# marcin-ochman/modular-slam

Hardware: AMD Instinct MI355X
Metric: ORB keypoints extracted+matched /sec, 640×480 RGB-D, 1/2/4/8 GPU; HBM GB/s vs roofline (higher is better)
Workload: dtype u8

## Files before the change

### include/mslam_hip.h

```cpp
#ifndef MSLAM_HIP_H_
#define MSLAM_HIP_H_

#include <stddef.h>
#include <stdint.h>

#ifdef __cplusplus
extern "C" {
#endif

#define MSLAM_HIP_ABI_VERSION 5

enum
{
    MSLAM_HIP_OK = 0,
    MSLAM_HIP_E_INVALID = 1,
    MSLAM_HIP_E_RUNTIME = 2,
    MSLAM_HIP_E_CAPACITY = 3,
    MSLAM_HIP_E_NO_VOCABULARY = 4,
    MSLAM_HIP_E_FORMAT = 5,
    MSLAM_HIP_E_NO_MODEL = 6
};

typedef struct mslam_hip_ctx mslam_hip_ctx;

// ... 327 lines not shown
                         int* best );

typedef struct
{
    int32_t n_matches, n_correspondences, n_inliers, status;
    double rvec[3], tvec[3], R[9];
    int32_t tracked;
    int32_t keyframe_required;
    int32_t keyframe_added;
    int32_t n_entry, n_inherited;
    int32_t vote_best, vote_best_count;
} mslam_hip_track_result;
int mslam_hip_track(mslam_hip_ctx* ctx, const uint8_t* desc, const float* xy, int n, const uint16_t* depth, int width,
                    int height, float factor, double fx, double fy, double cx, double cy, int ref_id,
                    const int32_t* vote_ids, int n_vote, double ratio, int iterations, double reprojection_error,
                    uint64_t seed, int use_extrinsic_guess, const double* rvec, const double* tvec,
                    int min_matched_points , int new_keyframe_min_landmarks , int new_id ,
                    double z_max , mslam_hip_track_result* out, int32_t* vote_counts ,
                    int32_t* pair_from, int32_t* pair_to, uint8_t* inliers, int pair_stride,
                    int32_t* entry_src, int32_t* entry_kp, int entry_capacity);

typedef mslam_hip_track_result mslam_hip_track_window_result;
int mslam_hip_track_window(mslam_hip_ctx* ctx, const uint8_t* desc, const float* xy, const int32_t* n, int stride,
                           const uint16_t* depth, int S, int width, int height, float factor, double fx, double fy, double cx,
                           double cy, int ref_id, const int32_t* vote_ids, int n_vote, int ref_vote_pos, double ratio,
                           int iterations, double reprojection_error, uint64_t seed, int use_extrinsic_guess,
                           const double* rvec, const double* tvec, int min_matched_points, int new_keyframe_min_landmarks,
                           int new_id, double z_max, mslam_hip_track_window_result* out , int* first_event,
                           int32_t* vote_counts , int32_t* entry_src, int32_t* entry_kp,
                           int entry_capacity);
int mslam_hip_track_window_dev(mslam_hip_ctx* ctx, int first_frame, int n_frames, double fx, double fy, double cx, double cy,
                               int ref_id, const int32_t* vote_ids, int n_vote, int ref_vote_pos, double ratio, int iterations,
                               double reprojection_error, uint64_t seed, int use_extrinsic_guess, const double* rvec,
                               const double* tvec, int min_matched_points, int new_keyframe_min_landmarks, int new_id,
                               double z_max, mslam_hip_track_window_result* out , int* first_event,
                               int32_t* vote_counts, int32_t* entry_src, int32_t* entry_kp, int entry_capacity);

enum
{
    MSLAM_HIP_DBG_PYRAMID = 0,
    MSLAM_HIP_DBG_BLURRED = 1,
    MSLAM_HIP_DBG_CANDIDATES = 2,
    MSLAM_HIP_DBG_SELECTED = 3,
    MSLAM_HIP_DBG_CELLS = 4,
    MSLAM_HIP_DBG_FORMS = 5,
    MSLAM_HIP_DBG_QUAD_DIRECT = 6
};
int mslam_hip_level_geometry(mslam_hip_ctx* ctx, int* widths, int* heights, float* scales);
int mslam_hip_debug_read(mslam_hip_ctx* ctx, int what, int frame, int level, void* dst, size_t dst_bytes,
                         size_t* n_items);

int mslam_hip_debug_counts(mslam_hip_ctx* ctx, int what, int32_t* out, int n_frames);

int mslam_hip_copy_to_host(mslam_hip_ctx* ctx, void* dst_host, const void* src_dev, size_t bytes);

int mslam_hip_set_profiling(mslam_hip_ctx* ctx, int enable);
int mslam_hip_get_stage_times(mslam_hip_ctx* ctx, const char** names, float* ms, int cap, int* n);

#ifdef __cplusplus
}
#endif
#endif
```

### modular-slam_amd/__init__.py

```python
import ctypes as C
import os
import subprocess

import numpy as np

_HERE = os.path.dirname(os.path.abspath(__file__))
LIB_PATH = os.path.join(_HERE, "libmslam_hip.so")

OK, E_INVALID, E_RUNTIME, E_CAPACITY, E_NO_VOCABULARY, E_FORMAT, E_NO_MODEL = range(7)
DBG_PYRAMID, DBG_BLURRED, DBG_CANDIDATES, DBG_SELECTED, DBG_CELLS, DBG_FORMS, DBG_QUAD_DIRECT = range(7)
QUAD_DIRECT_MAX_CANDIDATES = 1024
MATCHER_AUTO, MATCHER_POPCOUNT = 0, 1
DETECTOR_DISTRIBUTED, DETECTOR_CV_ORB = 0, 1
BOW_ASSIGN_TREE, BOW_ASSIGN_FLAT = 0, 1
CV_ORDER_LIBSTDCXX, CV_ORDER_RASTER = 0, 1
POSE_GRAPH_MAX_KEYFRAMES, POSE_GRAPH_MAX_EDGES = 1024, 65536
POSE_GRAPH_MAX_KEYFRAMES_SPARSE, POSE_GRAPH_MAX_ENVELOPE_BLOCKS = 16384, 1048576
PG_SOLVER_DENSE, PG_SOLVER_SPARSE = 0, 1
_PG_SOLVER_NAMES = {"dense": PG_SOLVER_DENSE, "sparse": PG_SOLVER_SPARSE}
PG_ORDER_NATURAL, PG_ORDER_RCM = 0, 1
BA_GLOBAL_MAX_KEYFRAMES, BA_GLOBAL_MAX_KEYFRAMES_SPARSE = 1024, 16384
BA_GLOBAL_SOLVER_DENSE, BA_GLOBAL_SOLVER_SPARSE = 0, 1
CULL_MAX_ENTRIES = 4096
BA_LOSS_NONE, BA_LOSS_HUBER, BA_LOSS_CAUCHY = 0, 1, 2
_BA_LOSS_NAMES = {"none": BA_LOSS_NONE, "huber": BA_LOSS_HUBER, "cauchy": BA_LOSS_CAUCHY}
UNION_DESC_RECENT, UNION_DESC_DISTINCTIVE = 0, 1
_UNION_DESC_NAMES = {"recent": UNION_DESC_RECENT, "distinctive": UNION_DESC_DISTINCTIVE}

ABI_SYMBOLS = [
    "mslam_hip_default_params", "mslam_hip_abi_version", "mslam_hip_create", "mslam_hip_destroy",
    "mslam_hip_last_error", "mslam_hip_sync", "mslam_hip_detect", "mslam_hip_detect_batch_dev",
    "mslam_hip_get_batch_view", "mslam_hip_match", "mslam_hip_match_knn2", "mslam_hip_match_batch_dev",
    "mslam_hip_bow_load", "mslam_hip_bow_info", "mslam_hip_bow_words", "mslam_hip_bow_transform",
    "mslam_hip_bow_score", "mslam_hip_bow_db_add", "mslam_hip_bow_db_query", "mslam_hip_bow_db_clear",
    "mslam_hip_bow_batch_dev", "mslam_hip_get_bow_view", "mslam_hip_bow_cross_score_dev", "mslam_hip_level_geometry", "mslam_hip_debug_read",
    "mslam_hip_set_profiling", "mslam_hip_get_stage_times", "mslam_hip_copy_to_host", "mslam_hip_backproject", "mslam_hip_backproject_batch_dev",
    "mslam_hip_get_points_view", "mslam_hip_set_matcher", "mslam_hip_get_matcher",
    "mslam_hip_bow_pack_dev", "mslam_hip_bow_cross_score_packed_dev", "mslam_hip_debug_counts",
    "mslam_hip_last_match_kernel",
    "mslam_hip_join_matcher", "mslam_hip_bow_db_remove", "mslam_hip_bow_set_assignment",
    "mslam_hip_bow_db_reserve", "mslam_hip_bow_db_size", "mslam_hip_qlz_decompress",
    "mslam_hip_pnp_ransac", "mslam_hip_pnp_batch_dev", "mslam_hip_get_pnp_view", "mslam_hip_pnp_set_confidence", "mslam_hip_pack_batch_dev", "mslam_hip_packed_capacity",
    "mslam_hip_set_cv_keypoint_order", "mslam_hip_pnp_min_mse", "mslam_hip_pnp_min_mse_batch_dev",
    "mslam_hip_kf_add", "mslam_hip_kf_add_from_batch_dev", "mslam_hip_kf_remove", "mslam_hip_kf_clear", "mslam_hip_kf_size",
    "mslam_hip_kf_reserve", "mslam_hip_kf_read", "mslam_hip_relocalize",
    "mslam_hip_kf_visible", "mslam_hip_track", "mslam_hip_track_window", "mslam_hip_track_window_dev",
    "mslam_hip_kf_add_ids", "mslam_hip_kf_read_ids", "mslam_hip_kf_covisible", "mslam_hip_kf_union", "mslam_hip_kf_union_dev",
    "mslam_hip_match_guided_knn2", "mslam_hip_match_guided", "mslam_hip_set_guided_match", "mslam_hip_get_guided_match",
    "mslam_hip_bundle_adjust", "mslam_hip_bundle_adjust_global", "mslam_hip_kf_update_world", "mslam_hip_pose_graph",
    "mslam_hip_kf_fuse_search", "mslam_hip_kf_replace_ids", "mslam_hip_kf_fuse",
    "mslam_hip_kf_fuse_search_multi", "mslam_hip_kf_fuse_multi",
    "mslam_hip_kf_remove_observations",
    "mslam_hip_kf_observers", "mslam_hip_kf_cull_search", "mslam_hip_kf_cull",
    "mslam_hip_kf_remove_landmarks", "mslam_hip_kf_cull_landmarks_search", "mslam_hip_kf_cull_landmarks",
    "mslam_hip_set_ba_loss", "mslam_hip_get_ba_loss",
    "mslam_hip_set_union_descriptor", "mslam_hip_get_union_descriptor",
    "mslam_hip_set_pose_graph_solver", "mslam_hip_get_pose_graph_solver", "mslam_hip_pose_graph_analyze",
    "mslam_hip_set_ba_global_solver", "mslam_hip_get_ba_global_solver", "mslam_hip_bundle_adjust_global_analyze",
]


class MslamHipError(RuntimeError):
    def __init__(self, code, msg):
        super().__init__("mslam_hip error %d: %s" % (code, msg))
        self.code = code


class Params(C.Structure):
    _fields_ = [("width", C.c_int32), ("height", C.c_int32), ("max_batch", C.c_int32), ("n_levels", C.c_int32),
                ("scale_factor", C.c_float), ("ini_fast_thr", C.c_int32), ("min_fast_thr", C.c_int32),
                ("min_node_area", C.c_uint32), ("max_keypoints", C.c_int32), ("max_candidates", C.c_int32),
                ("device", C.c_int32), ("stream", C.c_void_p), ("detector", C.c_int32), ("n_features", C.c_int32),
                ("edge_threshold", C.c_int32)]


class BatchView(C.Structure):
    _fields_ = [("n_frames", C.c_int32), ("capacity", C.c_int32), ("xy", C.c_void_p), ("desc", C.c_void_p),
                ("octave", C.c_void_p), ("angle", C.c_void_p), ("response", C.c_void_p), ("count", C.c_void_p),
                ("match_from", C.c_void_p), ("match_to", C.c_void_p), ("match_count", C.c_void_p)]


class PointsView(C.Structure):
    _fields_ = [("capacity", C.c_int32), ("xyz", C.c_void_p), ("valid", C.c_void_p)]


class PackedHeader(C.Structure):
    _fields_ = [("n_frames", C.c_int32), ("total_keypoints", C.c_int32), ("total_matches", C.c_int32), ("with_points", C.c_int32),
                ("off_kp_offset", C.c_uint64), ("off_match_offset", C.c_uint64), ("off_xy", C.c_uint64), ("off_desc", C.c_uint64),
                ("off_octave", C.c_uint64), ("off_angle", C.c_uint64), ("off_response", C.c_uint64), ("off_xyz", C.c_uint64),
                ("off_valid", C.c_uint64), ("off_match_from", C.c_uint64), ("off_match_to", C.c_uint64), ("bytes", C.c_uint64),
                ("fits", C.c_int32), ("pad", C.c_int32)]


def unpack_batch(buf):
    h = PackedHeader.from_buffer_copy(bytes(buf[:C.sizeof(PackedHeader)]))
    if not h.fits:
        raise MslamHipError(E_CAPACITY, "packed results need %d bytes" % h.bytes)
    nk, nm, nf = h.total_keypoints, h.total_matches, h.n_frames

    def arr(off, dt, n, *shape):
        return np.frombuffer(buf, dt, n, int(off)).reshape((-1,) + shape) if shape else np.frombuffer(buf, dt, n, int(off))
    out = {"n_frames": nf, "bytes": int(h.bytes),
           "kp_offset": arr(h.off_kp_offset, np.int32, nf + 1), "match_offset": arr(h.off_match_offset, np.int32, nf + 1),
           "xy": arr(h.off_xy, np.float32, 2 * nk, 2), "desc": arr(h.off_desc, np.uint8, 32 * nk, 32),
           "octave": arr(h.off_octave, np.int32, nk), "angle": arr(h.off_angle, np.float32, nk),
           "response": arr(h.off_response, np.float32, nk),
           "match_from": arr(h.off_match_from, np.int32, nm), "match_to": arr(h.off_match_to, np.int32, nm)}
    if h.with_points:
        out["xyz"] = arr(h.off_xyz, np.float64, 3 * nk, 3)
        out["valid"] = arr(h.off_valid, np.uint8, nk)
    return out
# ... 887 lines not shown
    def bow_pack_dev(self, k_max, d_out):
        self._chk(self.L.mslam_hip_bow_pack_dev(self._h, int(k_max), C.c_void_p(d_out)))

    def bow_cross_score_packed_dev(self, d_sets, n_sets, self_set, n_frames, k_max, d_scores, stream=None):
        self._chk(self.L.mslam_hip_bow_cross_score_packed_dev(self._h, C.c_void_p(d_sets), int(n_sets), int(self_set),
                                                              int(n_frames), int(k_max), C.c_void_p(d_scores),
                                                              C.c_void_p(stream)))

    def bow_view(self):
        v = BowView()
        self._chk(self.L.mslam_hip_get_bow_view(self._h, C.byref(v)))
        return v

    def level_geometry(self):
        n = self.params.n_levels
        w = (C.c_int * 16)()
        h = (C.c_int * 16)()
        s = (C.c_float * 16)()
        self._chk(self.L.mslam_hip_level_geometry(self._h, w, h, s))
        return list(w[:n]), list(h[:n]), np.array(s[:n], np.float32)

    def debug_image(self, what, frame, level):
        w, h, _ = self.level_geometry()
        out = np.empty((h[level], w[level]), np.uint8)
        n = C.c_size_t(0)
        self._chk(self.L.mslam_hip_debug_read(self._h, what, frame, level, _p(out), C.c_size_t(out.size), C.byref(n)))
        return out

    def debug_keypoints(self, what, frame, level):
        out = np.empty((self.params.max_candidates, 3), np.float32)
        n = C.c_size_t(0)
        self._chk(self.L.mslam_hip_debug_read(self._h, what, frame, level, _p(out), C.c_size_t(out.nbytes),
                                              C.byref(n)))
        return out[:n.value].copy()

    def debug_cells(self, level):
        out = np.empty((2048, 6), np.int32)
        n = C.c_size_t(0)
        self._chk(self.L.mslam_hip_debug_read(self._h, DBG_CELLS, 0, level, _p(out), C.c_size_t(out.nbytes),
                                              C.byref(n)))
        return out[:n.value].copy()

    def debug_forms(self):
        out = np.zeros(2, np.int32)
        n = C.c_size_t(0)
        self._chk(self.L.mslam_hip_debug_read(self._h, DBG_FORMS, 0, 0, _p(out), C.c_size_t(out.nbytes), C.byref(n)))
        return int(out[0]), int(out[1])

    def debug_quad_direct_levels(self):
        out = np.zeros(1, np.uint32)
        n = C.c_size_t(0)
        self._chk(self.L.mslam_hip_debug_read(self._h, DBG_QUAD_DIRECT, 0, 0, _p(out), C.c_size_t(out.nbytes), C.byref(n)))
        return [bool((int(out[0]) >> l) & 1) for l in range(self.params.n_levels)]

    def debug_counts(self, what, n_frames):
        out = np.zeros((max(n_frames, 1), self.params.n_levels), np.int32)
        self._chk(self.L.mslam_hip_debug_counts(self._h, int(what), _p(out), int(out.shape[0])))
        return out[:n_frames]

    def set_profiling(self, enable):
        self._chk(self.L.mslam_hip_set_profiling(self._h, int(enable)))

    def stage_times(self, cap=256):
        names = (C.c_char_p * cap)()
        ms = (C.c_float * cap)()
        n = C.c_int(0)
        self._chk(self.L.mslam_hip_get_stage_times(self._h, names, ms, cap, C.byref(n)))
        return [(names[i].decode(), ms[i]) for i in range(n.value)]


def qlz_decompress(data, n_packets, capacity=None):
    src = np.frombuffer(bytes(data), np.uint8)
    cap = capacity if capacity is not None else 10000 * n_packets + 16
    dst = np.empty(max(cap, 1), np.uint8)
    n = C.c_size_t(0)
    L = lib()
    L.mslam_hip_qlz_decompress.argtypes = [C.c_void_p, C.c_size_t, C.c_uint32, C.c_void_p, C.c_size_t, C.POINTER(C.c_size_t)]
    rc = L.mslam_hip_qlz_decompress(_p(src), src.size, int(n_packets), _p(dst), dst.size, C.byref(n))
    if rc != OK:
        raise MslamHipError(rc, "qlz_decompress failed")
    return dst[:n.value].tobytes()


class RgbFrame:

    def __init__(self, data, width, height):
        self.data = np.ascontiguousarray(data, np.uint8).reshape(height, width, 3)
        self.size = (width, height)


class OrbKeypoint:
    __slots__ = ("id", "coordinates", "descriptor")

    def __init__(self, id, coordinates, descriptor):
        self.id, self.coordinates, self.descriptor = id, coordinates, descriptor


class HipOrbDetector:

    def __init__(self, width=640, height=480, **kw):
        self.ctx = Context(width=width, height=height, **kw)

    def detect(self, sensorData):
        r = self.ctx.detect(sensorData.data)
        return [OrbKeypoint(i, (float(x), float(y)), d) for i, ((x, y), d) in enumerate(zip(r["xy"].astype(np.float64),
                                                                                          r["desc"]))]
# ... 801 lines not shown
```

### modular-slam_amd/csrc/api.hip

```cpp
#include "context.hpp"

#include <cfloat>
#include <climits>
#include <cmath>
#include <cstdio>
#include <cstring>
#include <cstdlib>
#include <algorithm>

using namespace mslam;

static thread_local std::string g_create_error;

#define ENTER(c)                                                                                                       \
    do                                                                                                                 \
    {                                                                                                                  \
        if(!(c))                                                                                                       \
            return MSLAM_HIP_E_INVALID;                                                                                \
        MSLAM_CHK(c, hipSetDevice((c)->p.device));                                                                     \
    } while(0)

static inline int cv_round_f(float v) { return (int)lrintf(v); }
static inline int cv_floor_f(float v)
{
// ... 1664 lines not shown
            out[3 * i + 1] = (float)kp_y(tmp[i]);
            out[3 * i + 2] = (float)kp_score(tmp[i]);
        }
        if(c->p.detector == MSLAM_HIP_DETECTOR_CV_ORB && !cand)
        {
            std::vector<float> resp(n);
            if(n)
                MSLAM_CHK(c, hipMemcpy(resp.data(), reinterpret_cast<const float*>(c->quad.best) + slot * (size_t)c->p.max_candidates,
                                       (size_t)n * 4, hipMemcpyDeviceToHost));
            for(uint32_t i = 0; i < n; ++i)
            {
                out[3 * i] += (float)kBorder;
                out[3 * i + 1] += (float)kBorder;
                out[3 * i + 2] = resp[i];
            }
        }
        return MSLAM_HIP_OK;
    }
    if(what == MSLAM_HIP_DBG_CELLS && c->p.detector == MSLAM_HIP_DETECTOR_DISTRIBUTED)
    {
        *n_items = (size_t)lv.n_cells;
        if(dst_bytes < (size_t)lv.n_cells * 24)
            return fail(c, MSLAM_HIP_E_CAPACITY, "debug_read: buffer too small");
        int32_t* out = static_cast<int32_t*>(dst);
        for(int i = 0; i < lv.n_cells; ++i)
        {
            const CellDesc& cd = c->cells[(size_t)lv.cell_base + i];
            const int32_t rec[6] = {cd.x0, cd.y0, cd.cw, cd.ch, cd.ox, cd.oy};
            std::memcpy(out + 6 * i, rec, sizeof(rec));
        }
        return MSLAM_HIP_OK;
    }
    if(what == MSLAM_HIP_DBG_FORMS)
    {
        *n_items = 2;
        if(dst_bytes < 8)
            return fail(c, MSLAM_HIP_E_CAPACITY, "debug_read: buffer too small");
        const int32_t rec[2] = {c->fused_levels, c->geom.blur_tiled};
        std::memcpy(dst, rec, sizeof(rec));
        return MSLAM_HIP_OK;
    }
    if(what == MSLAM_HIP_DBG_QUAD_DIRECT)
    {
        *n_items = 1;
        if(dst_bytes < 4)
            return fail(c, MSLAM_HIP_E_CAPACITY, "debug_read: buffer too small");
        const uint32_t m = c->p.detector == MSLAM_HIP_DETECTOR_DISTRIBUTED ? quad_direct_levels(c->geom) : 0u;
        std::memcpy(dst, &m, sizeof(m));
        return MSLAM_HIP_OK;
    }
    return fail(c, MSLAM_HIP_E_INVALID, "debug_read: unknown item");
}

int mslam_hip_debug_counts(mslam_hip_ctx* c, int what, int32_t* out, int n_frames)
{
    ENTER(c);
    if(c->p.width == 0 || !out || n_frames < 1 || (what != MSLAM_HIP_DBG_CANDIDATES && what != MSLAM_HIP_DBG_SELECTED))
        return fail(c, MSLAM_HIP_E_INVALID, "debug_counts: bad argument");
    MSLAM_CHK(c, hipStreamSynchronize(c->stream));
    const int rows = std::min(n_frames, std::max(c->n_last, 1));
    MSLAM_CHK(c, hipMemcpy(out, what == MSLAM_HIP_DBG_CANDIDATES ? c->quad.cand_cnt : c->quad.sel_cnt,
                           (size_t)rows * c->geom.n_levels * 4, hipMemcpyDeviceToHost));
    return MSLAM_HIP_OK;
}

int mslam_hip_copy_to_host(mslam_hip_ctx* c, void* dst_host, const void* src_dev, size_t bytes)
{
    ENTER(c);
    if(!dst_host || !src_dev)
        return fail(c, MSLAM_HIP_E_INVALID, "copy_to_host: null pointer");
    MSLAM_CHK(c, hipStreamSynchronize(c->stream_m));
    MSLAM_CHK(c, hipStreamSynchronize(c->stream));
    MSLAM_CHK(c, hipMemcpy(dst_host, src_dev, bytes, hipMemcpyDeviceToHost));
    return MSLAM_HIP_OK;
}

int mslam_hip_set_profiling(mslam_hip_ctx* c, int enable)
{
    if(!c)
        return MSLAM_HIP_E_INVALID;
    c->profiling = enable == 1;
    c->inplace_timing = enable == 2;
    c->timers_used = 0;
    return MSLAM_HIP_OK;
}

int mslam_hip_get_stage_times(mslam_hip_ctx* c, const char** names, float* ms, int cap, int* n)
{
    ENTER(c);
    if(!n)
        return fail(c, MSLAM_HIP_E_INVALID, "get_stage_times: null output");
    MSLAM_CHK(c, hipStreamSynchronize(c->stream_m));
    MSLAM_CHK(c, hipStreamSynchronize(c->stream));
    int k = 0;
    for(size_t i = 0; i < c->timers_used && k < cap; ++i, ++k)
    {
        float t = 0;
        MSLAM_CHK(c, hipEventElapsedTime(&t, c->timers[i].start, c->timers[i].stop));
        if(names)
            names[k] = c->timers[i].name;
        if(ms)
            ms[k] = t;
    }
    *n = k;
    if(c->inplace_timing)
        c->timers_used = 0;
// ... 5 lines not shown
```

### modular-slam_amd/csrc/common.hpp

```cpp
#pragma once
#include <hip/hip_runtime.h>
#include <cstdint>
#include <cstddef>

namespace mslam
{

constexpr int kMaxLevels = 16;
constexpr int kBorder = 19;
constexpr int kCell = 64;
constexpr int kOverlap = 6;
constexpr int kCellCap = 1024;

constexpr size_t al256(size_t x) { return (x + 255) & ~(size_t)255; }

struct LevelGeom
{
    int w, h;
    int pitch;
    int offset;
    float scale;
    int bw, bh;
    int cell_base;
    int n_cells;
// ... 54 lines not shown
    kFlagKpOverflow = 2u,
    kFlagQuadNoConverge = 4u,
    kFlagBowPackOverflow = 8u,
    kFlagDbFull = 16u,
    kFlagPackOverflow = 32u,
    kFlagUnionOverflow = 64u
};

void launch_gray(const uint8_t* d_bgr, uint8_t* d_pyr, const Geometry& g, int frame0, int n_frames, hipStream_t s);
void launch_resize(uint8_t* d_pyr, const Geometry& g, int level, const int32_t* d_xofs, const uint32_t* d_xcoef,
                   const int32_t* d_yofs, const uint32_t* d_ycoef, int frame0, int n_frames, hipStream_t s);
struct ResizeColArgs
{
    uint8_t* pyr;
    unsigned slab;
    int src_off, sh, spitch, dst_off, dw, dh, dpitch;
    const uint4* qt;
    const int32_t* yofs;
    const uint32_t* ycoef;
    int frame0, n_frames;
    int quads;
    float inv_quads;
    int R;
    int need_mask;
    int exact;
};
void launch_resize_col(const ResizeColArgs& a, hipStream_t s);
void launch_fast(const uint8_t* d_pyr, const Geometry& g, const CellDesc* d_cells, uint32_t* d_cell_cnt,
                 uint32_t* d_cell_kp, int ini_thr, int min_thr, int frame0, int n_frames, hipStream_t s);
void launch_denorm_selfcheck(uint32_t* d_out, hipStream_t s);
struct QuadArgs
{
    const uint32_t* cell_cnt;
    const uint32_t* cell_kp;
    uint32_t* cand;
    uint32_t* cand_cnt;
    uint32_t* sel;
    uint32_t* sel_cnt;
    uint32_t* kp_node;
    uint2* nodes_a;
    uint2* nodes_b;
    uint32_t* ncnt_a;
    uint32_t* ncnt_b;
    uint32_t* child_cnt;
    uint32_t* ninfo;
    uint32_t* best;
    uint32_t* flags;
    int cand_cap;
    unsigned min_size;
};
void launch_quadtree(const Geometry& g, const QuadArgs& a, int frame0, int n_frames, hipStream_t s);
int quad_depth_bound(const LevelGeom& lv, unsigned min_size);
unsigned quad_direct_levels(const Geometry& g);
struct BlurK
{
    uint32_t ta[3], tb[4], tc[4];
    uint32_t t01, t23, t45, t6;
};
BlurK make_blur_k();
struct GrayBlurArgs
{
    const uint8_t* bgr;
    uint8_t* pyr;
    uint8_t* blur;
    int W, H, pitch;
    unsigned slab;
    int n_frames, frame0;
    int quads;
    float inv_quads;
    int wide;
    int k6;
    int waves_per_xcd;
    int blur_tiled;
    BlurK bk;
};
void launch_gray_blur(const GrayBlurArgs& a, hipStream_t s);
struct ResizeBlurArgs
{
    uint8_t* pyr;
    uint8_t* blur;
    unsigned slab;
    int src_off, sh, spitch, dst_off, dw, dh, dpitch;
    const uint4* qt;
    const int32_t* yofs;
    const uint32_t* ycoef;
    int frame0, n_frames;
    int quads;
    float inv_quads;
    int wide;
    int k6;
    int need_mask;
    int exact;
    int waves_per_xcd;
    int blur_tiled;
    int always_load;
    BlurK bk;
};
void launch_resize_blur(const ResizeBlurArgs& a, hipStream_t s);
constexpr int kOctNeed = 0x48;
constexpr int kChainLevels = 8;
struct LevelChainArgs
{
    GrayBlurArgs g;
    ResizeBlurArgs lv[kChainLevels - 1];
    int n_lv;
    int G;
// ... 163 lines not shown
```

### modular-slam_amd/csrc/k_quadtree.hip

```cpp
#include "common.hpp"
#include <algorithm>
#include <cstdlib>

namespace mslam
{

constexpr int QT = 512;
constexpr int kSmallKp = 512, kSmallQT = 256;
constexpr int kMidKp = 1024, kMidQT = 512;
constexpr int kLdsKp = 2048;
constexpr int kMaxCellsPerLevel = 2048;
constexpr int kBigNodes = 4096;
constexpr int kBigKp = 12288;
constexpr int kBigMinPixels = 400000;
constexpr int kMaxInitNodes = 64;
constexpr int kDirectKp = 1024, kDirectQT = 256, kDirectSlots = 1365, kDirectMaxDepth = 10;
constexpr int kMaxPasses = 40;

struct Scan
{
    uint32_t wsum[QT / 64];
};

__device__ __forceinline__ uint32_t wave_incl_scan(uint32_t v)
{
    int x = (int)v;
    x += __builtin_amdgcn_update_dpp(0, x, 0x111, 0xF, 0xF, true);
    x += __builtin_amdgcn_update_dpp(0, x, 0x112, 0xF, 0xF, true);
    x += __builtin_amdgcn_update_dpp(0, x, 0x114, 0xF, 0xE, true);
    x += __builtin_amdgcn_update_dpp(0, x, 0x118, 0xF, 0xC, true);
    x += __builtin_amdgcn_update_dpp(0, x, 0x142, 0xA, 0xF, true);
    x += __builtin_amdgcn_update_dpp(0, x, 0x143, 0xC, 0xF, true);
    return (uint32_t)x;
}

template <int NT>
__device__ __forceinline__ uint32_t block_excl_scan(uint32_t v, Scan& s, uint32_t& total)
{
    const int lane = threadIdx.x & 63, wave = threadIdx.x >> 6;
    const uint32_t inc = wave_incl_scan(v);
    if(lane == 63)
        s.wsum[wave] = inc;
    __syncthreads();
    uint32_t base = 0, tot = 0;
#pragma unroll
    for(int w = 0; w < NT / 64; ++w)
    {
        const uint32_t x = s.wsum[w];
        if(w < wave)
            base += x;
        tot += x;
    }
    __syncthreads();
    total = tot;
    return base + inc - v;
}

template <int NT>
__device__ __forceinline__ void block_excl_scan2(uint32_t a, uint32_t b, Scan& s, Scan& s2, uint32_t& exa, uint32_t& exb,
                                                 uint32_t& tota, uint32_t& totb)
{
    const int lane = threadIdx.x & 63, wave = threadIdx.x >> 6;
    const uint32_t ia = wave_incl_scan(a), ib = wave_incl_scan(b);
    if(lane == 63)
    {
        s.wsum[wave] = ia;
        s2.wsum[wave] = ib;
    }
    __syncthreads();
    uint32_t ba = 0, bb = 0, ta = 0, tb = 0;
// ... 285 lines not shown
        const int i = base + tid;
        const uint32_t v = i < n_cells ? ccnt[i] : 0u;
        uint32_t tot;
        const uint32_t ex = block_excl_scan<NT>(v, scan, tot);
        if(i < n_cells)
            cell_off[i] = running + ex;
        running += tot;
    }
    if(tid == 0)
        cell_off[n_cells] = running;
    __syncthreads();
    return running;
}

__device__ __forceinline__ int quad_class(uint32_t N, int n_cells, unsigned classes)
{
    if((classes & 1u) && N <= (uint32_t)kSmallKp && n_cells <= 2 * kSmallKp - 1)
        return 0;
    if((classes & 2u) && N <= (uint32_t)kMidKp && n_cells <= 2 * kMidKp - 1)
        return 1;
    return 2;
}
template <int KP, int NT, int CLS>
__global__ __launch_bounds__(NT) __attribute__((amdgpu_waves_per_eu(CLS == 2 ? 4 : 8))) void k_quadtree(Geometry g, QuadArgs a, unsigned big_levels, unsigned direct_levels)
{
    __shared__ Scan scan, scan2;
    __shared__ uint32_t l_cand[KP];
    __shared__ uint2 l_nodes_a[KP], l_nodes_b[KP];
    __shared__ uint32_t l_cc[KP * 2];
    __shared__ uint16_t l_kp_node[KP], l_ncnt_a[KP], l_ncnt_b[KP], l_nbase[KP];
    __shared__ uint8_t l_ninfo[KP];
    __shared__ uint32_t init_cnt[kMaxInitNodes];
    __shared__ uint32_t init_pos[kMaxInitNodes];
    __shared__ uint32_t sh_n;
    constexpr int kCellsFit = 2 * KP - 1;
    static_assert(CLS != 2 || kCellsFit >= kMaxCellsPerLevel, "cell offsets must fit");
    const unsigned classes = big_levels >> 30;
    uint32_t* cell_off = reinterpret_cast<uint32_t*>(l_nodes_b);

    const int level = (int)((blockIdx.x + blockIdx.y) % (unsigned)g.n_levels);
    const size_t frame = blockIdx.y + g.frame0;
    const LevelGeom& lv = g.lv[level];
    const int tid = threadIdx.x;
    const size_t slot = frame * g.n_levels + level;
    const size_t cap = (size_t)a.cand_cap;
    uint32_t* cand = a.cand + slot * cap;
    uint32_t* sel = a.sel + slot * cap;

    const int n_cells = lv.n_cells;
    if(n_cells > kCellsFit)
        return;
    const uint32_t* ccnt = a.cell_cnt + frame * g.n_cells + lv.cell_base;
    const uint32_t N = quad_cell_offsets<NT>(ccnt, n_cells, cell_off, scan);
    if(((direct_levels >> level) & 1u) && N <= (uint32_t)kDirectKp)
        return;
    if(quad_class(N, n_cells, classes) != CLS)
        return;
    if(N > (uint32_t)a.cand_cap)
    {
        if(tid == 0)
        {
            atomicOr(a.flags, kFlagCandOverflow);
            a.cand_cnt[slot] = 0;
            a.sel_cnt[slot] = 0;
        }
        return;
    }
    if(tid == 0)
        a.cand_cnt[slot] = N;
    if(N == 0)
    {
        if(tid == 0)
            a.sel_cnt[slot] = 0;
        return;
    }
    if(N <= (uint32_t)KP)
        quad_run<LdsStore, NT>(g, a, lv, frame, slot, tid, N, n_cells, cell_off, l_cand, cand, l_kp_node, l_nodes_a, l_nodes_b,
                               l_ncnt_a, l_ncnt_b, l_ninfo, l_nbase, l_cc, l_cc, sel, scan, scan2, init_cnt, init_pos, sh_n);
    else if((big_levels >> level) & 1u)
        return;
    else
        quad_run<GlobalStore, NT>(g, a, lv, frame, slot, tid, N, n_cells, cell_off, cand, cand, a.kp_node + slot * cap,
                                  a.nodes_a + slot * cap, a.nodes_b + slot * cap, a.ncnt_a + slot * cap,
                                  a.ncnt_b + slot * cap, a.ninfo + slot * cap, a.best + slot * cap,
                                  a.child_cnt + slot * cap * 4, a.best + slot * cap, sel, scan, scan2, init_cnt, init_pos,
                                  sh_n);
}

__global__ __launch_bounds__(QT) void k_quadtree_big(Geometry g, QuadArgs a, unsigned big_levels)
{
    extern __shared__ __attribute__((aligned(16))) uint8_t big_lds[];
    __shared__ Scan scan, scan2;
    __shared__ uint32_t init_cnt[kMaxInitNodes];
    __shared__ uint32_t init_pos[kMaxInitNodes];
    __shared__ uint32_t sh_n;
    uint2* l_nodes_a = reinterpret_cast<uint2*>(big_lds);
    uint2* l_nodes_b = l_nodes_a + kBigNodes;
    uint32_t* l_cc = reinterpret_cast<uint32_t*>(l_nodes_b + kBigNodes);
    uint16_t* l_kp_node = reinterpret_cast<uint16_t*>(l_cc + 2 * kBigNodes);
    uint16_t* l_ncnt_a = l_kp_node + kBigKp;
    uint16_t* l_ncnt_b = l_ncnt_a + kBigNodes;
    uint16_t* l_nbase = l_ncnt_b + kBigNodes;
    uint8_t* l_ninfo = reinterpret_cast<uint8_t*>(l_nbase + kBigNodes);
    static_assert(kBigNodes * sizeof(uint2) >= (kMaxCellsPerLevel + 1) * sizeof(uint32_t), "cell offsets must fit");
    uint32_t* cell_off = reinterpret_cast<uint32_t*>(l_nodes_b);

    int level = 0;
    {
        unsigned m = big_levels;
        const unsigned which = (blockIdx.x + blockIdx.y) % gridDim.x;
        for(unsigned i = 0; i < which; ++i)
            m &= m - 1;
        level = __ffs((int)m) - 1;
    }
    const size_t frame = blockIdx.y + g.frame0;
    const LevelGeom& lv = g.lv[level];
    const int tid = threadIdx.x;
    const size_t slot = frame * g.n_levels + level;
    const size_t cap = (size_t)a.cand_cap;
    uint32_t* cand = a.cand + slot * cap;
    uint32_t* sel = a.sel + slot * cap;
    const int n_cells = lv.n_cells;
    const uint32_t* ccnt = a.cell_cnt + frame * g.n_cells + lv.cell_base;
    const uint32_t N = quad_cell_offsets<QT>(ccnt, n_cells, cell_off, scan);
    if(N <= (uint32_t)kLdsKp || N > (uint32_t)a.cand_cap)
        return;
    bool done = false;
    if(N <= (uint32_t)kBigKp)
        done = quad_run<BigStore, QT>(g, a, lv, frame, slot, tid, N, n_cells, cell_off, cand, cand, l_kp_node, l_nodes_a, l_nodes_b,
                                  l_ncnt_a, l_ncnt_b, l_ninfo, l_nbase, l_cc, l_cc, sel, scan, scan2, init_cnt, init_pos, sh_n);
    if(!done)
    {
        __syncthreads();
        quad_cell_offsets<QT>(ccnt, n_cells, cell_off, scan);
        quad_run<GlobalStore, QT>(g, a, lv, frame, slot, tid, N, n_cells, cell_off, cand, cand, a.kp_node + slot * cap,
                              a.nodes_a + slot * cap, a.nodes_b + slot * cap, a.ncnt_a + slot * cap,
                              a.ncnt_b + slot * cap, a.ninfo + slot * cap, a.best + slot * cap,
                              a.child_cnt + slot * cap * 4, a.best + slot * cap, sel, scan, scan2, init_cnt, init_pos,
                              sh_n);
    }
}

template <int SLOTS>
struct DirectTable
{
    uint32_t cnt[(SLOTS + 1) / 2];
    uint32_t best[SLOTS];
    uint8_t flag[SLOTS];
};

__device__ __forceinline__ uint32_t direct_block_start(uint32_t n_init, int d) { return n_init * (((1u << (2 * d)) - 1u) / 3u); }

template <int KP, int SLOTS, int NT>
__global__ __launch_bounds__(NT) __attribute__((amdgpu_waves_per_eu(8))) void k_quadtree_direct(Geometry g, QuadArgs a, unsigned direct_levels)
{
    constexpr int PER = KP / NT;
    static_assert(KP % NT == 0 && KP == kDirectKp, "instance shape");
    __shared__ Scan scan;
    __shared__ uint32_t l_cand[KP];
    __shared__ DirectTable<SLOTS> t;
    __shared__ uint32_t tot[2 * (kDirectMaxDepth + 2)];

    const int level = (int)((blockIdx.x + blockIdx.y) % (unsigned)g.n_levels);
    if(!((direct_levels >> level) & 1u))
        return;
    const size_t frame = blockIdx.y + g.frame0;
    const LevelGeom& lv = g.lv[level];
    const int tid = threadIdx.x;
    const size_t slot = frame * g.n_levels + level;
    const size_t cap = (size_t)a.cand_cap;
    uint32_t* g_cand = a.cand + slot * cap;
    uint32_t* sel = a.sel + slot * cap;
    const int D = lv.qdepth;
    const uint32_t n_init = (uint32_t)(lv.nxg * lv.nyg);
    const uint32_t n_slots = direct_block_start(n_init, D + 1);

    for(uint32_t i = tid; i < (n_slots + 1) / 2; i += NT)
        t.cnt[i] = 0;
    for(uint32_t i = tid; i < n_slots; i += NT)
        t.flag[i] = 0;
    if(tid < 2 * (kDirectMaxDepth + 2))
        tot[tid] = 0;

    const int n_cells = lv.n_cells;
    uint32_t* cell_off = t.best;
    const uint32_t* ccnt = a.cell_cnt + frame * g.n_cells + lv.cell_base;
    const uint32_t N = quad_cell_offsets<NT>(ccnt, n_cells, cell_off, scan);
    if(N > (uint32_t)KP)
        return;
    if(N > (uint32_t)a.cand_cap)
    {
        if(tid == 0)
        {
            atomicOr(a.flags, kFlagCandOverflow);
            a.cand_cnt[slot] = 0;
            a.sel_cnt[slot] = 0;
        }
        return;
    }
    if(tid == 0)
        a.cand_cnt[slot] = N;
    if(N == 0)
    {
        if(tid == 0)
            a.sel_cnt[slot] = 0;
        return;
    }

    const uint32_t* ckp = a.cell_kp + (frame * g.n_cells + lv.cell_base) * (size_t)kCellCap;
    const float sf = lv.scale;
    const float min_size_f = (float)a.min_size;
    uint32_t path[PER];
#pragma unroll
    for(int i = 0; i < PER; ++i)
    {
        const uint32_t k = (uint32_t)(tid + i * NT);
        path[i] = ~0u;
        if(k >= N)
            continue;
        int lo = 0, hi = n_cells - 1;
        while(lo < hi)
        {
            const int mid = (lo + hi + 1) >> 1;
            if(cell_off[mid] <= k)
                lo = mid;
            else
                hi = mid - 1;
        }
        const uint32_t p = ckp[(size_t)lo * kCellCap + (k - cell_off[lo])];
        l_cand[k] = p;
        g_cand[k] = p;
        const int x = kp_x(p), y = kp_y(p);
        const unsigned ix = (unsigned)((double)(float)x / lv.delta_x);
        const unsigned iy = (unsigned)((double)(float)y / lv.delta_y);
        const unsigned idx = ix + iy * (unsigned)lv.nxg;
        if(idx >= n_init)
            continue;
        int bx = (int)(lv.delta_x * ix), by = (int)(lv.delta_y * iy);
        int ex = (int)(lv.delta_x * (ix + 1)), ey = (int)(lv.delta_y * (iy + 1));
        uint32_t q = idx;
        int d = 0;
        for(;;)
        {
            const uint32_t s = direct_block_start(n_init, d) + q;
            atomicAdd(&t.cnt[s >> 1], 1u << (16 * (s & 1u)));
            const unsigned area = (unsigned)((ex - bx) * (ey - by));
            if(__fmul_rn(__fmul_rn((float)area, sf), sf) <= min_size_f || d == D)
            {
                t.flag[s] = 1;
                break;
            }
            const int cx = bx + ((ex - bx + 1) >> 1), cy = by + ((ey - by + 1) >> 1);
            const bool right = cx <= x, low = cy <= y;
            bx = right ? cx : bx, ex = right ? ex : cx;
            by = low ? cy : by, ey = low ? ey : cy;
            q = (q << 2) | (right ? 1u : 0u) | (low ? 2u : 0u);
            ++d;
        }
        path[i] = ((uint32_t)d << 24) | q;
    }
    __syncthreads();

    for(int d = 0; d <= D; ++d)
    {
        const uint32_t start = direct_block_start(n_init, d), n_d = n_init << (2 * d);
        const uint32_t pstart = direct_block_start(n_init, d > 0 ? d - 1 : 0);
        uint32_t kd = 0, md = 0;
        for(uint32_t base = 0; base < n_d; base += NT)
        {
            const uint32_t q = base + tid;
            bool keep = false, open = false;
            if(q < n_d)
            {
                const uint32_t s = start + q, ps = pstart + (q >> 2);
                const uint32_t c = (t.cnt[s >> 1] >> (16 * (s & 1u))) & 0xFFFFu;
                const uint32_t pc = d > 0 ? (t.cnt[ps >> 1] >> (16 * (ps & 1u))) & 0xFFFFu : 2u;
                const bool real = c > 0 && pc >= 2;
                keep = real && (c == 1 || t.flag[s] != 0);
                open = real && !keep;
                t.flag[s] = keep ? 1 : open ? 2 : 0;
                t.best[s] = 0;
            }
            kd += (uint32_t)__popcll(__ballot(keep));
            md += (uint32_t)__popcll(__ballot(open));
        }
        if((tid & 63) == 0 && (kd | md) != 0)
        {
            atomicAdd(&tot[2 * d], kd);
            atomicAdd(&tot[2 * d + 1], md);
        }
    }
    __syncthreads();
    int P = 1;
    while(tot[2 * P] + tot[2 * P + 1] != tot[2 * P - 1])
        ++P;
    const int top = P < D ? P : D;

#pragma unroll
    for(int i = 0; i < PER; ++i)
    {
        if(path[i] == ~0u)
            continue;
        const uint32_t k = (uint32_t)(tid + i * NT);
        const int dk = (int)(path[i] >> 24);
        const uint32_t q = path[i] & 0xFFFFFFu;
        const int last = dk < top ? dk : top;
        uint32_t leaf = 0;
        for(int d = 0; d <= last; ++d)
        {
            leaf = direct_block_start(n_init, d) + (q >> (2 * (dk - d)));
            if(t.flag[leaf] == 1)
                break;
        }
        atomicMax(&t.best[leaf], ((uint32_t)kp_score(l_cand[k]) << 24) | (0xFFFFFFu - k));
    }
    __syncthreads();

    const uint32_t n_entries = direct_block_start(n_init, top + 1);
    const uint32_t per = (n_entries + NT - 1) / NT;
    const uint32_t e0 = (uint32_t)tid * per, e1 = e0 + per < n_entries ? e0 + per : n_entries;
    auto entry_slot = [&](uint32_t e, bool& is_leaf) {
        int d = top;
        uint32_t n_d = n_init << (2 * d);
        while(e >= n_d)
        {
            e -= n_d;
            --d;
            n_d >>= 2;
        }
        const uint32_t bits = 2u * (uint32_t)d, low_mask = (1u << bits) - 1u;
        uint32_t i0 = e >> bits;
        if(d & 1)
            i0 = n_init - 1u - i0;
        const uint32_t s = direct_block_start(n_init, d) + ((i0 << bits) | ((e ^ 0x33333333u) & low_mask));
        const uint32_t f = t.flag[s];
        is_leaf = f == 1 || (f == 2 && d == P);
        return s;
    };
    uint32_t mine = 0;
    for(uint32_t e = e0; e < e1; ++e)
    {
        bool is_leaf;
        entry_slot(e, is_leaf);
        mine += is_leaf ? 1u : 0u;
    }
    uint32_t n_leaves;
    uint32_t r = block_excl_scan<NT>(mine, scan, n_leaves);
    for(uint32_t e = e0; e < e1 && mine != 0; ++e)
    {
        bool is_leaf;
        const uint32_t s = entry_slot(e, is_leaf);
        if(is_leaf)
            sel[r++] = l_cand[0xFFFFFFu - (t.best[s] & 0xFFFFFFu)];
    }
    if(tid == 0)
        a.sel_cnt[slot] = n_leaves;
}

unsigned quad_direct_levels(const Geometry& g)
{
    const char* env = getenv("MSLAM_HIP_QUAD_DIRECT");
    const bool on = !env || atoi(env) != 0;
    unsigned m = 0;
    for(int l = 0; on && l < g.n_levels; ++l)
    {
        const LevelGeom& lv = g.lv[l];
        if(lv.qdepth < 0 || lv.qdepth > kDirectMaxDepth || lv.n_cells + 1 > kDirectSlots)
            continue;
        const long long slots = (long long)lv.nxg * lv.nyg * (((1ll << (2 * (lv.qdepth + 1))) - 1) / 3);
        if(slots <= kDirectSlots)
            m |= 1u << l;
    }
    return m;
}

int quad_depth_bound(const LevelGeom& lv, unsigned min_size)
{
    int dx = 0, dy = 0;
    for(int iy = 0; iy < lv.nyg; ++iy)
        for(int ix = 0; ix < lv.nxg; ++ix)
        {
            dx = std::max(dx, (int)(lv.delta_x * (ix + 1)) - (int)(lv.delta_x * ix));
            dy = std::max(dy, (int)(lv.delta_y * (iy + 1)) - (int)(lv.delta_y * iy));
        }
    for(int d = 0; d <= 15; ++d)
    {
        const unsigned area = (unsigned)(dx * dy);
        const float scaled = (float)area * lv.scale;
        if(scaled * lv.scale <= (float)min_size)
            return d;
        if(dx <= 1 && dy <= 1)
            break;
        dx = (dx + 1) >> 1, dy = (dy + 1) >> 1;
    }
    return -1;
}

void launch_quadtree(const Geometry& g, const QuadArgs& a, int frame0, int n_frames, hipStream_t s)
{
    dim3 grid(g.n_levels, n_frames);
    Geometry gg = g;
    gg.frame0 = frame0;
    unsigned big_levels = 0;
    for(int l = 0; l < g.n_levels; ++l)
        if(g.lv[l].w * g.lv[l].h > kBigMinPixels)
            big_levels |= 1u << l;
    static const unsigned classes_env = [] { const char* e = getenv("MSLAM_HIP_QUAD_CLASSES"); return e ? (unsigned)atoi(e) & 3u : 3u; }();
    const unsigned direct = quad_direct_levels(g);
    const bool all_direct = direct == (g.n_levels >= 32 ? ~0u : (1u << g.n_levels) - 1u);
    const unsigned classes = n_frames < 8 || all_direct ? 0u : classes_env;
    const unsigned bl = big_levels | (classes << 30);
    if(direct != 0)
        hipLaunchKernelGGL((k_quadtree_direct<kDirectKp, kDirectSlots, kDirectQT>), grid, dim3(kDirectQT), 0, s, gg, a, direct);
    hipLaunchKernelGGL((k_quadtree<kLdsKp, QT, 2>), grid, dim3(QT), 0, s, gg, a, bl, direct);
    if(classes & 2u)
        hipLaunchKernelGGL((k_quadtree<kMidKp, kMidQT, 1>), grid, dim3(kMidQT), 0, s, gg, a, bl, direct);
    if(classes & 1u)
        hipLaunchKernelGGL((k_quadtree<kSmallKp, kSmallQT, 0>), grid, dim3(kSmallQT), 0, s, gg, a, bl, direct);
    if(big_levels != 0)
    {
        constexpr size_t lds = (size_t)kBigNodes * (8 + 8 + 8 + 2 + 2 + 2 + 1) + (size_t)kBigKp * 2;
        static const bool attr = [] {
            return hipFuncSetAttribute((const void*)k_quadtree_big, hipFuncAttributeMaxDynamicSharedMemorySize, (int)lds) == hipSuccess;
        }();
        (void)attr;
        hipLaunchKernelGGL(k_quadtree_big, dim3((unsigned)__builtin_popcount(big_levels), n_frames), dim3(QT), lds, s, gg, a,
                           big_levels);
    }
}

}
```

Measured before the change: 685.0 million.

## Let direct quadtree kernel handle overflow candidates, skip fallback launches when all-direct

The direct quadtree kernel now handles levels with more than its LDS capacity of candidates. It spills the overflow candidates' quadtree paths to global memory, then votes and selects from global storage. When every level is direct and the candidate capacity fits the direct count limit, the launcher skips the large, mid, small and big fallback kernels entirely, which saves launches and early-exit blocks. The cost is some global-memory traffic for overflow keypoints. A debug API is added to report the launch plan.

```diff
diff --git a/include/mslam_hip.h b/include/mslam_hip.h
--- a/include/mslam_hip.h
+++ b/include/mslam_hip.h
@@ -403,6 +403,16 @@
 
 int mslam_hip_debug_counts(mslam_hip_ctx* ctx, int what, int32_t* out, int n_frames);
 
+enum
+{
+    MSLAM_HIP_QUAD_KERNEL_DIRECT = 1,
+    MSLAM_HIP_QUAD_KERNEL_LARGE = 2,
+    MSLAM_HIP_QUAD_KERNEL_MID = 4,
+    MSLAM_HIP_QUAD_KERNEL_SMALL = 8,
+    MSLAM_HIP_QUAD_KERNEL_BIG = 16
+};
+int mslam_hip_debug_quad_launch_plan(mslam_hip_ctx* ctx, int n_frames, uint32_t* kernels);
+
 int mslam_hip_copy_to_host(mslam_hip_ctx* ctx, void* dst_host, const void* src_dev, size_t bytes);
 
 int mslam_hip_set_profiling(mslam_hip_ctx* ctx, int enable);
diff --git a/modular-slam_amd/__init__.py b/modular-slam_amd/__init__.py
--- a/modular-slam_amd/__init__.py
+++ b/modular-slam_amd/__init__.py
@@ -10,6 +10,8 @@
 OK, E_INVALID, E_RUNTIME, E_CAPACITY, E_NO_VOCABULARY, E_FORMAT, E_NO_MODEL = range(7)
 DBG_PYRAMID, DBG_BLURRED, DBG_CANDIDATES, DBG_SELECTED, DBG_CELLS, DBG_FORMS, DBG_QUAD_DIRECT = range(7)
 QUAD_DIRECT_MAX_CANDIDATES = 1024
+QUAD_DIRECT_COUNT_LIMIT = 65535
+QUAD_KERNEL_NAMES = ("direct", "large", "mid", "small", "big")
 MATCHER_AUTO, MATCHER_POPCOUNT = 0, 1
 DETECTOR_DISTRIBUTED, DETECTOR_CV_ORB = 0, 1
 BOW_ASSIGN_TREE, BOW_ASSIGN_FLAT = 0, 1
@@ -57,6 +59,7 @@
     "mslam_hip_set_union_descriptor", "mslam_hip_get_union_descriptor",
     "mslam_hip_set_pose_graph_solver", "mslam_hip_get_pose_graph_solver", "mslam_hip_pose_graph_analyze",
     "mslam_hip_set_ba_global_solver", "mslam_hip_get_ba_global_solver", "mslam_hip_bundle_adjust_global_analyze",
+    "mslam_hip_debug_quad_launch_plan",
 ]
 
 
@@ -1050,6 +1053,11 @@
         n = C.c_size_t(0)
         self._chk(self.L.mslam_hip_debug_read(self._h, DBG_QUAD_DIRECT, 0, 0, _p(out), C.c_size_t(out.nbytes), C.byref(n)))
         return [bool((int(out[0]) >> l) & 1) for l in range(self.params.n_levels)]
+
+    def debug_quad_launch_plan(self, n_frames):
+        m = C.c_uint32(0)
+        self._chk(self.L.mslam_hip_debug_quad_launch_plan(self._h, int(n_frames), C.byref(m)))
+        return [name for b, name in enumerate(QUAD_KERNEL_NAMES) if (m.value >> b) & 1]
 
     def debug_counts(self, what, n_frames):
         out = np.zeros((max(n_frames, 1), self.params.n_levels), np.int32)
diff --git a/modular-slam_amd/csrc/api.hip b/modular-slam_amd/csrc/api.hip
--- a/modular-slam_amd/csrc/api.hip
+++ b/modular-slam_amd/csrc/api.hip
@@ -1740,6 +1740,19 @@
     return fail(c, MSLAM_HIP_E_INVALID, "debug_read: unknown item");
 }
 
+int mslam_hip_debug_quad_launch_plan(mslam_hip_ctx* c, int n_frames, uint32_t* kernels)
+{
+    ENTER(c);
+    if(c->p.width == 0 || !kernels || n_frames < 1)
+        return fail(c, MSLAM_HIP_E_INVALID, "debug_quad_launch_plan: bad argument");
+    static_assert(MSLAM_HIP_QUAD_KERNEL_DIRECT == kQuadKernelDirect && MSLAM_HIP_QUAD_KERNEL_LARGE == kQuadKernelLarge &&
+                      MSLAM_HIP_QUAD_KERNEL_MID == kQuadKernelMid && MSLAM_HIP_QUAD_KERNEL_SMALL == kQuadKernelSmall &&
+                      MSLAM_HIP_QUAD_KERNEL_BIG == kQuadKernelBig,
+                  "the header's bits are the launcher's");
+    *kernels = c->p.detector == MSLAM_HIP_DETECTOR_DISTRIBUTED ? quad_launch_plan(c->geom, c->quad.cand_cap, n_frames).kernels : 0u;
+    return MSLAM_HIP_OK;
+}
+
 int mslam_hip_debug_counts(mslam_hip_ctx* c, int what, int32_t* out, int n_frames)
 {
     ENTER(c);
diff --git a/modular-slam_amd/csrc/common.hpp b/modular-slam_amd/csrc/common.hpp
--- a/modular-slam_amd/csrc/common.hpp
+++ b/modular-slam_amd/csrc/common.hpp
@@ -130,6 +130,22 @@
 void launch_quadtree(const Geometry& g, const QuadArgs& a, int frame0, int n_frames, hipStream_t s);
 int quad_depth_bound(const LevelGeom& lv, unsigned min_size);
 unsigned quad_direct_levels(const Geometry& g);
+enum : unsigned
+{
+    kQuadKernelDirect = 1u,
+    kQuadKernelLarge = 2u,
+    kQuadKernelMid = 4u,
+    kQuadKernelSmall = 8u,
+    kQuadKernelBig = 16u
+};
+struct QuadPlan
+{
+    unsigned kernels;
+    unsigned direct_levels;
+    unsigned big_levels;
+    unsigned classes;
+};
+QuadPlan quad_launch_plan(const Geometry& g, int cand_cap, int n_frames);
 struct BlurK
 {
     uint32_t ta[3], tb[4], tc[4];
diff --git a/modular-slam_amd/csrc/k_quadtree.hip b/modular-slam_amd/csrc/k_quadtree.hip
--- a/modular-slam_amd/csrc/k_quadtree.hip
+++ b/modular-slam_amd/csrc/k_quadtree.hip
@@ -15,7 +15,13 @@
 constexpr int kBigMinPixels = 400000;
 constexpr int kMaxInitNodes = 64;
 constexpr int kDirectKp = 1024, kDirectQT = 256, kDirectSlots = 1365, kDirectMaxDepth = 10;
+constexpr uint32_t kDirectCountLimit = 0xFFFFu;
 constexpr int kMaxPasses = 40;
+
+__host__ __device__ __forceinline__ bool quad_direct_owns(uint32_t N, int cand_cap)
+{
+    return N <= (uint32_t)cand_cap && N <= kDirectCountLimit;
+}
 
 struct Scan
 {
@@ -407,7 +413,7 @@
         return;
     const uint32_t* ccnt = a.cell_cnt + frame * g.n_cells + lv.cell_base;
     const uint32_t N = quad_cell_offsets<NT>(ccnt, n_cells, cell_off, scan);
-    if(((direct_levels >> level) & 1u) && N <= (uint32_t)kDirectKp)
+    if(((direct_levels >> level) & 1u) && quad_direct_owns(N, a.cand_cap))
         return;
     if(quad_class(N, n_cells, classes) != CLS)
         return;
@@ -442,7 +448,7 @@
                                   sh_n);
 }
 
-__global__ __launch_bounds__(QT) void k_quadtree_big(Geometry g, QuadArgs a, unsigned big_levels)
+__global__ __launch_bounds__(QT) void k_quadtree_big(Geometry g, QuadArgs a, unsigned big_levels, unsigned direct_levels)
 {
     extern __shared__ __attribute__((aligned(16))) uint8_t big_lds[];
     __shared__ Scan scan, scan2;
@@ -480,6 +486,8 @@
     const uint32_t N = quad_cell_offsets<QT>(ccnt, n_cells, cell_off, scan);
     if(N <= (uint32_t)kLdsKp || N > (uint32_t)a.cand_cap)
         return;
+    if(((direct_levels >> level) & 1u) && quad_direct_owns(N, a.cand_cap))
+        return;
     bool done = false;
     if(N <= (uint32_t)kBigKp)
         done = quad_run<BigStore, QT>(g, a, lv, frame, slot, tid, N, n_cells, cell_off, cand, cand, l_kp_node, l_nodes_a, l_nodes_b,
@@ -511,6 +519,7 @@
 {
     constexpr int PER = KP / NT;
     static_assert(KP % NT == 0 && KP == kDirectKp, "instance shape");
+    static_assert(kDirectCountLimit == 0xFFFFu, "DirectTable::cnt packs two 16-bit counters into a dword");
     __shared__ Scan scan;
     __shared__ uint32_t l_cand[KP];
     __shared__ DirectTable<SLOTS> t;
@@ -525,6 +534,7 @@
     const size_t slot = frame * g.n_levels + level;
     const size_t cap = (size_t)a.cand_cap;
     uint32_t* g_cand = a.cand + slot * cap;
+    uint32_t* g_path = a.kp_node + slot * cap;
     uint32_t* sel = a.sel + slot * cap;
     const int D = lv.qdepth;
     const uint32_t n_init = (uint32_t)(lv.nxg * lv.nyg);
@@ -541,8 +551,6 @@
     uint32_t* cell_off = t.best;
     const uint32_t* ccnt = a.cell_cnt + frame * g.n_cells + lv.cell_base;
     const uint32_t N = quad_cell_offsets<NT>(ccnt, n_cells, cell_off, scan);
-    if(N > (uint32_t)KP)
-        return;
     if(N > (uint32_t)a.cand_cap)
     {
         if(tid == 0)
@@ -553,6 +561,8 @@
         }
         return;
     }
+    if(!quad_direct_owns(N, a.cand_cap))
+        return;
     if(tid == 0)
         a.cand_cnt[slot] = N;
     if(N == 0)
@@ -565,14 +575,7 @@
     const uint32_t* ckp = a.cell_kp + (frame * g.n_cells + lv.cell_base) * (size_t)kCellCap;
     const float sf = lv.scale;
     const float min_size_f = (float)a.min_size;
-    uint32_t path[PER];
-#pragma unroll
-    for(int i = 0; i < PER; ++i)
-    {
-        const uint32_t k = (uint32_t)(tid + i * NT);
-        path[i] = ~0u;
-        if(k >= N)
-            continue;
+    auto descend = [&](uint32_t k, bool in_lds) -> uint32_t {
         int lo = 0, hi = n_cells - 1;
         while(lo < hi)
         {
@@ -583,14 +586,15 @@
                 hi = mid - 1;
         }
         const uint32_t p = ckp[(size_t)lo * kCellCap + (k - cell_off[lo])];
-        l_cand[k] = p;
+        if(in_lds)
+            l_cand[k] = p;
         g_cand[k] = p;
         const int x = kp_x(p), y = kp_y(p);
         const unsigned ix = (unsigned)((double)(float)x / lv.delta_x);
         const unsigned iy = (unsigned)((double)(float)y / lv.delta_y);
         const unsigned idx = ix + iy * (unsigned)lv.nxg;
         if(idx >= n_init)
-            continue;
+            return ~0u;
         int bx = (int)(lv.delta_x * ix), by = (int)(lv.delta_y * iy);
         int ex = (int)(lv.delta_x * (ix + 1)), ey = (int)(lv.delta_y * (iy + 1));
         uint32_t q = idx;
@@ -612,8 +616,17 @@
             q = (q << 2) | (right ? 1u : 0u) | (low ? 2u : 0u);
             ++d;
         }
-        path[i] = ((uint32_t)d << 24) | q;
-    }
+        return ((uint32_t)d << 24) | q;
+    };
+    uint32_t path[PER];
+#pragma unroll
+    for(int i = 0; i < PER; ++i)
+    {
+        const uint32_t k = (uint32_t)(tid + i * NT);
+        path[i] = k < N ? descend(k, true) : ~0u;
+    }
+    for(uint32_t k = (uint32_t)(KP + tid); k < N; k += NT)
+        g_path[k] = descend(k, false);
     __syncthreads();
 
     for(int d = 0; d <= D; ++d)
@@ -651,14 +664,9 @@
         ++P;
     const int top = P < D ? P : D;
 
-#pragma unroll
-    for(int i = 0; i < PER; ++i)
-    {
-        if(path[i] == ~0u)
-            continue;
-        const uint32_t k = (uint32_t)(tid + i * NT);
-        const int dk = (int)(path[i] >> 24);
-        const uint32_t q = path[i] & 0xFFFFFFu;
+    auto vote = [&](uint32_t k, uint32_t pth, uint32_t word) {
+        const int dk = (int)(pth >> 24);
+        const uint32_t q = pth & 0xFFFFFFu;
         const int last = dk < top ? dk : top;
         uint32_t leaf = 0;
         for(int d = 0; d <= last; ++d)
@@ -667,7 +675,20 @@
             if(t.flag[leaf] == 1)
                 break;
         }
-        atomicMax(&t.best[leaf], ((uint32_t)kp_score(l_cand[k]) << 24) | (0xFFFFFFu - k));
+        atomicMax(&t.best[leaf], ((uint32_t)kp_score(word) << 24) | (0xFFFFFFu - k));
+    };
+#pragma unroll
+    for(int i = 0; i < PER; ++i)
+    {
+        const uint32_t k = (uint32_t)(tid + i * NT);
+        if(path[i] != ~0u)
+            vote(k, path[i], l_cand[k]);
+    }
+    for(uint32_t k = (uint32_t)(KP + tid); k < N; k += NT)
+    {
+        const uint32_t pth = g_path[k];
+        if(pth != ~0u)
+            vote(k, pth, g_cand[k]);
     }
     __syncthreads();
 
@@ -706,7 +727,10 @@
         bool is_leaf;
         const uint32_t s = entry_slot(e, is_leaf);
         if(is_leaf)
-            sel[r++] = l_cand[0xFFFFFFu - (t.best[s] & 0xFFFFFFu)];
+        {
+            const uint32_t k = 0xFFFFFFu - (t.best[s] & 0xFFFFFFu);
+            sel[r++] = k < (uint32_t)KP ? l_cand[k] : g_cand[k];
+        }
     }
     if(tid == 0)
         a.sel_cnt[slot] = n_leaves;
@@ -751,28 +775,42 @@
     return -1;
 }
 
+QuadPlan quad_launch_plan(const Geometry& g, int cand_cap, int n_frames)
+{
+    QuadPlan p = {};
+    for(int l = 0; l < g.n_levels; ++l)
+        if(g.lv[l].w * g.lv[l].h > kBigMinPixels)
+            p.big_levels |= 1u << l;
+    static const unsigned classes_env = [] { const char* e = getenv("MSLAM_HIP_QUAD_CLASSES"); return e ? (unsigned)atoi(e) & 3u : 3u; }();
+    p.direct_levels = quad_direct_levels(g);
+    const bool all_direct = p.direct_levels == (g.n_levels >= 32 ? ~0u : (1u << g.n_levels) - 1u);
+    if(p.direct_levels != 0)
+        p.kernels |= kQuadKernelDirect;
+    if(all_direct && quad_direct_owns((uint32_t)cand_cap, cand_cap))
+        return p;
+    p.classes = n_frames < 8 || all_direct ? 0u : classes_env;
+    p.kernels |= kQuadKernelLarge | (p.classes & 2u ? kQuadKernelMid : 0u) | (p.classes & 1u ? kQuadKernelSmall : 0u) |
+                 (p.big_levels != 0 ? kQuadKernelBig : 0u);
+    return p;
+}
+
 void launch_quadtree(const Geometry& g, const QuadArgs& a, int frame0, int n_frames, hipStream_t s)
 {
     dim3 grid(g.n_levels, n_frames);
     Geometry gg = g;
     gg.frame0 = frame0;
-    unsigned big_levels = 0;
-    for(int l = 0; l < g.n_levels; ++l)
-        if(g.lv[l].w * g.lv[l].h > kBigMinPixels)
-            big_levels |= 1u << l;
-    static const unsigned classes_env = [] { const char* e = getenv("MSLAM_HIP_QUAD_CLASSES"); return e ? (unsigned)atoi(e) & 3u : 3u; }();
-    const unsigned direct = quad_direct_levels(g);
-    const bool all_direct = direct == (g.n_levels >= 32 ? ~0u : (1u << g.n_levels) - 1u);
-    const unsigned classes = n_frames < 8 || all_direct ? 0u : classes_env;
-    const unsigned bl = big_levels | (classes << 30);
-    if(direct != 0)
+    const QuadPlan p = quad_launch_plan(g, a.cand_cap, n_frames);
+    const unsigned direct = p.direct_levels, big_levels = p.big_levels;
+    const unsigned bl = big_levels | (p.classes << 30);
+    if(p.kernels & kQuadKernelDirect)
         hipLaunchKernelGGL((k_quadtree_direct<kDirectKp, kDirectSlots, kDirectQT>), grid, dim3(kDirectQT), 0, s, gg, a, direct);
-    hipLaunchKernelGGL((k_quadtree<kLdsKp, QT, 2>), grid, dim3(QT), 0, s, gg, a, bl, direct);
-    if(classes & 2u)
+    if(p.kernels & kQuadKernelLarge)
+        hipLaunchKernelGGL((k_quadtree<kLdsKp, QT, 2>), grid, dim3(QT), 0, s, gg, a, bl, direct);
+    if(p.kernels & kQuadKernelMid)
         hipLaunchKernelGGL((k_quadtree<kMidKp, kMidQT, 1>), grid, dim3(kMidQT), 0, s, gg, a, bl, direct);
-    if(classes & 1u)
+    if(p.kernels & kQuadKernelSmall)
         hipLaunchKernelGGL((k_quadtree<kSmallKp, kSmallQT, 0>), grid, dim3(kSmallQT), 0, s, gg, a, bl, direct);
-    if(big_levels != 0)
+    if(p.kernels & kQuadKernelBig)
     {
         constexpr size_t lds = (size_t)kBigNodes * (8 + 8 + 8 + 2 + 2 + 2 + 1) + (size_t)kBigKp * 2;
         static const bool attr = [] {
@@ -780,8 +818,8 @@
         }();
         (void)attr;
         hipLaunchKernelGGL(k_quadtree_big, dim3((unsigned)__builtin_popcount(big_levels), n_frames), dim3(QT), lds, s, gg, a,
-                           big_levels);
-    }
-}
-
-}
+                           big_levels, direct);
+    }
+}
+
+}
```

Result: no change. 683.6 million (-0.2%).
